# fdarmon/wild_deep_mvs

Hardware: AMD Instinct MI355X
Metric: cost-volume voxels/sec (BxDxHxW), MVSNet hot path (higher is better)
Workload: dtype bf16

## Files before the change

wild_deep_mvs_amd/csrc/conv3d.hip:

```cpp
#include "conv_common.h"
#include <type_traits>

namespace pscv {

PSCV_PROF_BUFFER(conv)

struct ConvArgs : ConvIO {
    int Di, Hi, Wi, Do, Ho, Wo;
    int cout, epi;
    int ntd, nth, ntw;
    unsigned mg_td, mg_th, mg_tw;
    int nt_total;
};

template <int KIND, int TD, int TH> struct Brick;
template <int TD, int TH> struct Brick<PSCV_CONV_S1, TD, TH> { static constexpr int BD = TD + 2, BH = TH + 2, BW = 18; };
template <int TD, int TH> struct Brick<PSCV_CONV_S2, TD, TH> { static constexpr int BD = 2 * TD + 1, BH = 2 * TH + 1, BW = 33; };
template <int TD, int TH> struct Brick<PSCV_CONV_T2, TD, TH> { static constexpr int BD = TD + 1, BH = TH + 1, BW = 17; };

__host__ __device__ constexpr int ceil_div(int a, int b) { return (a + b - 1) / b; }
__host__ __device__ constexpr int t2_ntaps(int pc) { return (1 + ((pc >> 2) & 1)) * (1 + ((pc >> 1) & 1)) * (1 + (pc & 1)); }
__host__ __device__ constexpr int t2_nsteps(int pc, int cin) { return ceil_div(t2_ntaps(pc) * cin, 32); }
__host__ __device__ constexpr int t2_stepbase(int pc, int cin) {
    int s = 0;
    for (int i = 0; i < pc; ++i) s += t2_nsteps(i, cin);
    return s;
}
__host__ __device__ constexpr int conv_total_steps(int kind, int cin) {
    return kind == PSCV_CONV_T2 ? t2_stepbase(8, cin) : ceil_div(27 * cin, 32);
}

__host__ __device__ constexpr int conv_vs(int kind, int cin, int th = 4) {
    if (kind == PSCV_CONV_S1 && cin == 64 && th == 8) return 144;
    if (kind == PSCV_CONV_S2) return cin == 32 ? 80 : cin * 2 + 16;
    return cin == 16 ? 32 : cin == 8 ? 48 : cin * 2 + 32;
}
__host__ __device__ constexpr int conv_epi_bytes(int nt) { return 3 * nt * 16 * 4; }

__host__ __device__ constexpr int conv_region0(int kind, int cin, int nt, int td, int th) {
    const int bd = kind == PSCV_CONV_S1 ? td + 2 : kind == PSCV_CONV_S2 ? 2 * td + 1 : td + 1;
    const int bh = kind == PSCV_CONV_S1 ? th + 2 : kind == PSCV_CONV_S2 ? 2 * th + 1 : th + 1;
    const int bw = kind == PSCV_CONV_S1 ? 18 : kind == PSCV_CONV_S2 ? 33 : 17;
    const int brick = (bd * bh * bw * conv_vs(kind, cin, th) + 15) & ~15;
    const int red = (td * th == 4 && kind != PSCV_CONV_T2) ? 16 * 1024 * nt : 0;
    return brick > red ? brick : red;
}

template <int KIND, int BH, int BW, int VS> __device__ __forceinline__ int tap_off_dense(int tap) {
    tap = tap > 26 ? 26 : tap;
    const int kd = tap / 9, kh = (tap / 3) % 3, kw = tap % 3;
    return ((kd * BH + kh) * BW + kw) * VS;
}
template <int BH, int BW, int VS> __device__ __forceinline__ int tap_off_t2(int pc, int t) {
    const int pd = (pc >> 2) & 1, ph = (pc >> 1) & 1, pw = pc & 1;
    const int nt = (1 + pd) * (1 + ph) * (1 + pw);
    t = t >= nt ? nt - 1 : t;
    const int tw = t % (1 + pw), th = (t / (1 + pw)) % (1 + ph), td = t / ((1 + pw) * (1 + ph));
    const int od = (pd && td == 0) ? 1 : 0, oh = (ph && th == 0) ? 1 : 0, ow = (pw && tw == 0) ? 1 : 0;
    return ((od * BH + oh) * BW + ow) * VS;
}

template <typename H>
__device__ __noinline__ void epi_ragged(float y0, float y1, float y2, float y3, const uint16_t* sp, void* op, int cnt, int out_f32,
                                        float lo_post) {
    float y[4] = {y0, y1, y2, y3};
    for (int k = 0; k < cnt; ++k) {
        float v = y[k];
        if (sp) v += Half16<H>::one(sp[k]);
        v = relu_floor(v, lo_post);
        if (out_f32) reinterpret_cast<float*>(op)[k] = v;
        else reinterpret_cast<uint16_t*>(op)[k] = Half16<H>::bits(v);
    }
}

template <typename H, int CIN, int NT, int KIND, int TD, int TH>
__global__ __launch_bounds__(256) void conv3d_kernel(const ConvArgs a) {
    using BR = Brick<KIND, TD, TH>;
    constexpr int BD = BR::BD, BH = BR::BH, BW = BR::BW;
    constexpr int VS = conv_vs(KIND, CIN, TH);
    constexpr int CCH = CIN / 8;
    constexpr int NVOX = BD * BH * BW;
    constexpr int NMT = TD * TH;
    constexpr int MB = NMT / 4;
    static_assert(NMT % 4 == 0, "tile rows must split evenly over the 4 waves");
    constexpr int SXY = (KIND == PSCV_CONV_S2) ? 2 : 1;

    extern __shared__ __attribute__((aligned(16))) unsigned char smem[];
    PSCV_PROF_BEGIN

    int wg = xcd_remap(blockIdx.x, gridDim.x);
    const int tw_i = fast_divmod(wg, a.ntw, a.mg_tw);
    const int th_i = fast_divmod(wg, a.nth, a.mg_th);
    const int td_i = fast_divmod(wg, a.ntd, a.mg_td);
    const int b = wg;

    const int t0d = td_i * TD, t0h = th_i * TH, t0w = tw_i * 16;
    const int o_d = (KIND == PSCV_CONV_S1) ? t0d - 1 : (KIND == PSCV_CONV_S2) ? 2 * t0d - 1 : t0d;
    const int o_h = (KIND == PSCV_CONV_S1) ? t0h - 1 : (KIND == PSCV_CONV_S2) ? 2 * t0h - 1 : t0h;
    const int o_w = (KIND == PSCV_CONV_S1) ? t0w - 1 : (KIND == PSCV_CONV_S2) ? 2 * t0w - 1 : t0w;

    const int tid = threadIdx.x;
    const int lane = tid & 63, wave = __builtin_amdgcn_readfirstlane(tid >> 6);
    const int n = lane & 15, g = lane >> 4;
    const int nt0 = blockIdx.y * NT;
    const uint4* wpk = reinterpret_cast<const uint4*>(a.wpk);
    constexpr int NSTEPS_ALL = conv_total_steps(KIND, CIN);
    constexpr bool KSPLIT = MB == 1 && KIND != PSCV_CONV_T2;
    constexpr bool CSPLIT = MB == 1 && KIND == PSCV_CONV_T2;
    constexpr int SPW = (NSTEPS_ALL + 3) / 4;
    constexpr int PF_WANT = 24 / NT;
    constexpr int PF_SRC = KSPLIT ? SPW : NSTEPS_ALL;
    constexpr int PF = (KIND == PSCV_CONV_T2) ? 1 : (PF_SRC < PF_WANT ? PF_SRC : PF_WANT);
    uint4 wring[PF][NT];
    if (KIND != PSCV_CONV_T2) {
#pragma unroll
        for (int s = 0; s < PF; ++s) {
            int st = KSPLIT ? wave + 4 * s : s;
            st = st < NSTEPS_ALL ? st : NSTEPS_ALL - 1;
#pragma unroll
            for (int m = 0; m < NT; ++m) wring[s][m] = wpk[(st * a.nt_total + nt0 + m) * 64 + lane];
        }
    }
    constexpr int CS_MAXW = CSPLIT ? t2_nsteps(0, CIN) + t2_nsteps(7, CIN) : 1;
    uint4 wcls[CS_MAXW][NT];
    uint2 skc[CSPLIT ? 8 : 1][NT];
    constexpr int XS = KIND == PSCV_CONV_T2 ? 2 : 1;
    const int ox0 = XS * (t0w + n);
    const int cg = nt0 * 16 + g * 4;
    const unsigned lane_out = (unsigned)(ox0 * a.out_cs + cg), lane_skip = (unsigned)(ox0 * a.skip_cs + cg);
    const bool lane_ok = t0w + n < (KIND == PSCV_CONV_T2 ? a.Wi : a.Wo);
    const long plane_out = (long)a.Ho * a.Wo * a.out_cs, plane_skip = (long)a.Ho * a.Wo * a.skip_cs;
    const int row_out = a.Wo * a.out_cs, row_skip = a.Wo * a.skip_cs;
    const int bDo = b * a.Do;
    const bool cout4 = (a.cout & 3) == 0;
    auto out_row = [&](int od, int oh) -> long { return (long)(bDo + od) * plane_out + (long)oh * row_out + a.out_co; };
    auto skip_row = [&](int od, int oh) -> long { return (long)(bDo + od) * plane_skip + (long)oh * row_skip + a.skip_co; };
    auto skip_fetch = [&](long srow, int pw, int m) -> uint2 {
        uint2 sv = make_uint2(0u, 0u);
        if (a.skip && cout4) {
            if (lane_ok && cg + m * 16 < a.cout)
                sv = *reinterpret_cast<const uint2*>(a.skip + srow + (lane_skip + (unsigned)(pw * a.skip_cs + m * 16)));
        }
        return sv;
    };
    const long cs_orow0 = CSPLIT ? out_row(2 * t0d, 2 * t0h) : 0, cs_srow0 = CSPLIT ? skip_row(2 * t0d, 2 * t0h) : 0;
    auto cls_fetch = [&](auto pcc, auto woffc, auto soffc) {
        constexpr int pc = decltype(pcc)::value, WOFF = decltype(woffc)::value, SOFF = decltype(soffc)::value;
        constexpr int nsteps = t2_nsteps(pc, CIN), sbase = t2_stepbase(pc, CIN);
#pragma unroll
        for (int s = 0; s < nsteps; ++s)
#pragma unroll
            for (int m = 0; m < NT; ++m) wcls[WOFF + s][m] = wpk[((sbase + s) * a.nt_total + nt0 + m) * 64 + lane];
        constexpr int pd = (pc >> 2) & 1, ph = (pc >> 1) & 1, pw = pc & 1;
#pragma unroll
        for (int i = 0; i < 4; ++i) {
            const int id = t0d + i / TH, ih = t0h + i % TH;
            const bool in_ok = id < a.Di && ih < a.Hi;
#pragma unroll
            for (int m = 0; m < NT; ++m)
                skc[SOFF + i][m] = in_ok ? skip_fetch(cs_srow0 + (pd ? plane_skip : 0) + (2 * i + ph) * row_skip, pw, m) : make_uint2(0u, 0u);
        }
    };
    if constexpr (CSPLIT) {
        using std::integral_constant;
#define PSCV_CLS_PAIR(W) case W: cls_fetch(integral_constant<int, W>{}, integral_constant<int, 0>{}, integral_constant<int, 0>{}); \
                             cls_fetch(integral_constant<int, 7 - W>{}, integral_constant<int, t2_nsteps(W, CIN)>{}, integral_constant<int, 4>{}); break;
        switch (wave) { PSCV_CLS_PAIR(0) PSCV_CLS_PAIR(1) PSCV_CLS_PAIR(2) default: PSCV_CLS_PAIR(3) }
#undef PSCV_CLS_PAIR
    }
    uint2 skk[NT];
    if constexpr (KSPLIT) {
#pragma unroll
        for (int m = 0; m < NT; ++m) {
            const int od = t0d + wave / TH, oh = t0h + wave % TH;
            skk[m] = (od < a.Do && oh < a.Ho) ? skip_fetch(skip_row(od, oh), 0, m) : make_uint2(0u, 0u);
        }
    }
    PSCV_STAMP(5)

    {
        constexpr int PC = BH * BW * CCH;
        constexpr int NS = (PC + 255) / 256;
        constexpr int PG = (16 / NS) < 1 ? 1 : ((16 / NS) > BD ? BD : (16 / NS));
        const unsigned long plane_bytes = (unsigned long)a.Hi * a.Wi * a.in_cs * 2;
        const char* inb = reinterpret_cast<const char*>(a.in + (long)b * a.Di * a.Hi * a.Wi * a.in_cs + a.in_co);
        unsigned goff[NS];
        int lds_off[NS];
        bool ok[NS];
#pragma unroll
        for (int sl = 0; sl < NS; ++sl) {
            const int c = sl * 256 + tid;
            const int v = c / CCH, cc = c - v * CCH;
            const int bh = v / BW, bw = v - bh * BW;
            const int gh = o_h + bh, gw = o_w + bw;
            ok[sl] = c < PC && (unsigned)gh < (unsigned)a.Hi && (unsigned)gw < (unsigned)a.Wi;
            goff[sl] = ok[sl] ? (unsigned)(gh * a.Wi + gw) * (unsigned)(a.in_cs * 2) + (unsigned)(cc * 16) : 0u;
            lds_off[sl] = c < PC ? v * VS + cc * 16 : -1;
        }
#pragma unroll
        for (int p0 = 0; p0 < BD; p0 += PG) {
            uint4 val[PG][NS];
#pragma unroll
            for (int pp = 0; pp < PG; ++pp) {
                const int gd = o_d + p0 + pp;
                const bool pv = p0 + pp < BD && (unsigned)gd < (unsigned)a.Di;
                const char* pb = inb + (unsigned long)(pv ? gd : 0) * plane_bytes;
#pragma unroll
                for (int sl = 0; sl < NS; ++sl) {
                    val[pp][sl] = make_uint4(0u, 0u, 0u, 0u);
                    if (pv && ok[sl]) val[pp][sl] = *reinterpret_cast<const uint4*>(pb + goff[sl]);
                }
            }
            PSCV_STAMP(0)
            PSCV_STAMP_WAIT(1)
// ... 217 lines not shown
                    const int koff = tap_off_t2<BH, BW, VS>(pc, kk0 / CIN) + (kk0 % CIN) * 2;
                    const int fs = sbase + s;
                    uint4 wf[NT];
#pragma unroll
                    for (int m = 0; m < NT; ++m) wf[m] = wpk[(fs * a.nt_total + nt0 + m) * 64 + lane];
#pragma unroll
                    for (int i = 0; i < MB; ++i) {
                        const uint4 xf = *reinterpret_cast<const uint4*>(smem + anchor[i] + koff);
#pragma unroll
                        for (int m = 0; m < NT; ++m) acc[i][m] = Mfma<H>::run(wf[m], xf, acc[i][m]);
                    }
                }
            }
            PSCV_STAMP(3)
#pragma unroll
            for (int i = 0; i < MB; ++i) {
                const int mt = wave * MB + i;
                const int id = t0d + mt / TH, ih = t0h + mt % TH;
                if (id < a.Di && ih < a.Hi) epilogue(acc[i], 2 * id + pd, 2 * ih + ph, pw, skp[i]);
            }
            PSCV_STAMP(4)
        }
    }
    PSCV_STAMP_WAIT(5)
    PSCV_PROF_END(conv, blockIdx.x + gridDim.x * blockIdx.y)
}

template <typename H, int CIN, int NT, int KIND, int TD, int TH>
static int launch_conv(ConvArgs& a, int n_split, hipStream_t st) {
    constexpr int LDS = conv_region0(KIND, CIN, NT, TD, TH) + conv_epi_bytes(NT);
    static_assert(LDS <= 160 * 1024, "brick does not fit the 160 KiB LDS");
    const int rd = KIND == PSCV_CONV_T2 ? a.Di : a.Do, rh = KIND == PSCV_CONV_T2 ? a.Hi : a.Ho,
              rw = KIND == PSCV_CONV_T2 ? a.Wi : a.Wo;
    a.ntd = ceil_div(rd, TD); a.nth = ceil_div(rh, TH); a.ntw = ceil_div(rw, 16);
    const long nblk = finish_grid("pscv_conv3d", a.B, a.ntd, a.nth, a.ntw, a.mg_td, a.mg_th, a.mg_tw);
    if (nblk < 0) return -1;
    return launch("pscv_conv3d", conv3d_kernel<H, CIN, NT, KIND, TD, TH>, dim3((unsigned)nblk, (unsigned)n_split), dim3(256), LDS, st, a);
}

template <typename H, int CIN, int NT>
static int launch_kind(ConvArgs& a, int kind, hipStream_t st) {
    a.nt_total = NT;
    const int rd = kind == PSCV_CONV_T2 ? a.Di : a.Do, rh = kind == PSCV_CONV_T2 ? a.Hi : a.Ho,
              rw = kind == PSCV_CONV_T2 ? a.Wi : a.Wo;
    const int TDb = kind == PSCV_CONV_S1 ? 4 : 2, THb = kind == PSCV_CONV_S2 ? 2 : 4;
    const long big = (long)a.B * ceil_div(rd, TDb) * ceil_div(rh, THb) * ceil_div(rw, 16);
    const bool small = big < 1024 && g_conv_small_tiles && kind != PSCV_CONV_S2;
    const int want = (int)g_conv_small_nt;
    auto nts_of = [&](int dflt) { return (want == 1 || want == 2 || want == 4) && want <= NT && NT % want == 0 ? want : dflt; };
#define PSCV_NTS_SWITCH(NTSV, KINDV, TDV, THV)                                                                     \
    switch (NTSV) {                                                                                                  \
        case 1: return launch_conv<H, CIN, 1, KINDV, TDV, THV>(a, NT, st);                                           \
        case 2: if constexpr (NT >= 2) return launch_conv<H, CIN, 2, KINDV, TDV, THV>(a, NT / 2, st); break;         \
        default: if constexpr (NT >= 4) return launch_conv<H, CIN, 4, KINDV, TDV, THV>(a, NT / 4, st); break;        \
    }
    switch (kind) {
        case PSCV_CONV_S1:
            if (small) { PSCV_NTS_SWITCH(nts_of(NT == 2 ? 2 : 1), PSCV_CONV_S1, 1, 4) }
            if constexpr (CIN == 64) {
                if (g_conv_tall64 == 2 || (g_conv_tall64 && (long)a.B * ceil_div(rd, 4) * ceil_div(rh, 8) * ceil_div(rw, 16) >= 256))
                    return launch_conv<H, CIN, NT, PSCV_CONV_S1, 4, 8>(a, 1, st);
            }
            return launch_conv<H, CIN, NT, PSCV_CONV_S1, 4, 4>(a, 1, st);
        case PSCV_CONV_S2: { PSCV_NTS_SWITCH(nts_of(NT), PSCV_CONV_S2, 2, 2) } break;
        case PSCV_CONV_T2:
            if (small) { PSCV_NTS_SWITCH(nts_of(1), PSCV_CONV_T2, 1, 4) }
            return launch_conv<H, CIN, NT, PSCV_CONV_T2, 2, 4>(a, 1, st);
    }
#undef PSCV_NTS_SWITCH
    set_error("pscv_conv3d: unknown kind %d", kind);
    return -1;
}

template <typename H>
static int launch_channels(ConvArgs& a, int c_in, int c_out, int kind, hipStream_t st) {
    const int nt = (c_out + 15) / 16;
#define PSCV_CONV_CASE(CI, NTV) if (c_in == CI && nt == NTV) return launch_kind<H, CI, NTV>(a, kind, st);
    PSCV_CONV_CASE(8, 1) PSCV_CONV_CASE(8, 2)
    PSCV_CONV_CASE(16, 1) PSCV_CONV_CASE(16, 2)
    PSCV_CONV_CASE(32, 1) PSCV_CONV_CASE(32, 2) PSCV_CONV_CASE(32, 4)
    PSCV_CONV_CASE(64, 2) PSCV_CONV_CASE(64, 4)
#undef PSCV_CONV_CASE
    set_error("pscv_conv3d: unsupported channel combination c_in=%d c_out=%d", c_in, c_out);
    return -1;
}

}

PSCV_PROF_EXPORT(conv)

extern "C" int pscv_conv3d_cat2(const void* in_a, int a_cstride, int a_coff, const void* in_b, int b_cstride, int b_coff, int dtype,
                                const uint16_t* packed, const float* scale, const float* bias, const float* floor, const void* skip,
                                int skip_cstride, int skip_coff, void* out, int out_cstride, int out_coff, int out_dtype, int B, int D,
                                int H, int W, int c_out, int epi_flags, void* stream) {
    using namespace pscv;
    PSCV_CHECK_ARG(in_a && in_b && packed && out, "pscv_conv3d_cat2: null pointer argument");
    PSCV_CHECK_ARG(B > 0 && D > 0 && H > 0 && W > 0, "pscv_conv3d_cat2: bad sizes");
    PSCV_CHECK_ARG(c_out == 8 || c_out == 16, "pscv_conv3d_cat2: c_out=%d must be 8 or 16", c_out);
    PSCV_CHECK_ARG(a_cstride % 8 == 0 && a_coff % 8 == 0 && a_coff + 8 <= a_cstride && b_cstride % 8 == 0 && b_coff % 8 == 0 && b_coff + 8 <= b_cstride,
                   "pscv_conv3d_cat2: both inputs contribute an 8-aligned slice of 8 channels");
    PSCV_CHECK_ARG(out_coff + c_out <= out_cstride && out_cstride % 4 == 0 && out_coff % 4 == 0, "pscv_conv3d_cat2: bad output channel slice");
    PSCV_CHECK_ARG(!skip || (skip_cstride % 4 == 0 && skip_coff % 4 == 0), "pscv_conv3d_cat2: skip slice must be 4-aligned");
    PSCV_CHECK_ARG(dtype == PSCV_BF16 || dtype == PSCV_F16, "pscv_conv3d_cat2: storage dtype %d must be bf16 or fp16", dtype);
    PSCV_CHECK_ARG(out_dtype == dtype || out_dtype == PSCV_F32, "pscv_conv3d_cat2: out dtype %d must be the storage dtype or fp32", out_dtype);
    ConvCall c{};
    c.io = {reinterpret_cast<const uint16_t*>(in_a), packed, scale, bias, floor, reinterpret_cast<const uint16_t*>(skip), out,
            a_cstride, a_coff, skip_cstride, skip_coff, out_cstride, out_coff, out_dtype == PSCV_F32, B};
    c.dtype = dtype; c.D = D; c.H = H; c.W = W; c.c_in = 16; c.c_out = c_out; c.epi = epi_flags;
    c.st = reinterpret_cast<hipStream_t>(stream);
    c.in2 = reinterpret_cast<const uint16_t*>(in_b); c.in2_cs = b_cstride; c.in2_co = b_coff;
    return conv3d_sweepc_launch(c);
}

extern "C" int pscv_conv3d(const void* in, int dtype, int in_cstride, int in_coff, const uint16_t* packed, const float* scale,
                           const float* bias, const float* floor, const void* skip, int skip_cstride, int skip_coff,
                           void* out, int out_cstride, int out_coff, int out_dtype, int B, int Di, int Hi, int Wi,
                           int c_in, int c_out, int kind, int epi_flags, void* stream) {
    using namespace pscv;
    PSCV_CHECK_ARG(in && packed && out, "pscv_conv3d: null pointer argument");
    PSCV_CHECK_ARG(B > 0 && Di > 0 && Hi > 0 && Wi > 0, "pscv_conv3d: bad sizes");
    PSCV_CHECK_ARG(in_cstride % 8 == 0 && in_coff % 8 == 0 && in_coff + c_in <= in_cstride,
                   "pscv_conv3d: input channel slice [%d,%d) of stride %d must be 8-aligned", in_coff, in_coff + c_in, in_cstride);
    PSCV_CHECK_ARG(out_coff + c_out <= out_cstride, "pscv_conv3d: output channel slice exceeds stride");
    PSCV_CHECK_ARG(c_out < 4 || (out_cstride % 4 == 0 && out_coff % 4 == 0), "pscv_conv3d: output slice must be 4-aligned");
    PSCV_CHECK_ARG(!skip || c_out < 4 || (skip_cstride % 4 == 0 && skip_coff % 4 == 0), "pscv_conv3d: skip slice must be 4-aligned");
    PSCV_CHECK_ARG(dtype == PSCV_BF16 || dtype == PSCV_F16, "pscv_conv3d: storage dtype %d must be bf16 or fp16", dtype);
    PSCV_CHECK_ARG(out_dtype == dtype || out_dtype == PSCV_F32, "pscv_conv3d: out dtype %d must be the storage dtype or fp32", out_dtype);
    ConvCall c{};
    c.io = {reinterpret_cast<const uint16_t*>(in), packed, scale, bias, floor, reinterpret_cast<const uint16_t*>(skip), out,
            in_cstride, in_coff, skip_cstride, skip_coff, out_cstride, out_coff, out_dtype == PSCV_F32, B};
    c.dtype = dtype; c.D = Di; c.H = Hi; c.W = Wi; c.c_in = c_in; c.c_out = c_out; c.epi = epi_flags;
    c.st = reinterpret_cast<hipStream_t>(stream);
    if (kind == PSCV_CONV_S1P8) {
        PSCV_CHECK_ARG(((c_in == 8 || c_in == 16 || c_in == 32) && c_out == 8) || (c_in == 16 && c_out == 16),
                       "pscv_conv3d: the sweep kernels (S1P8) are for 8|16|32 -> 8 and 16 -> 16 (got %d -> %d)", c_in, c_out);
        return c_in == 32 ? conv3d_sweep8_launch(c) : conv3d_sweepc_launch(c);
    }
    if (kind == PSCV_CONV_T2P8) {
        PSCV_CHECK_ARG(c_in == 16 && c_out == 8, "pscv_conv3d: the parity-pair kernel (T2P8) is for c_in=16, c_out=8 (got %d -> %d)", c_in, c_out);
        return conv3d_t2p8_launch(c);
    }
    if (kind == PSCV_CONV_S1C1) {
        PSCV_CHECK_ARG(c_out == 1 && (c_in == 8 || c_in == 16), "pscv_conv3d: the 1-channel kernel (S1C1) is for c_in 8/16 -> 1 (got %d -> %d)", c_in, c_out);
        return conv3d_c1_launch(c);
    }
    if (kind == PSCV_CONV_S2) {
        const int rc = conv3d_sweep_s2_launch(c);
        if (rc != 1) return rc;
    }
    if (kind == PSCV_CONV_S1) {
        const int rc = conv3d_wide_launch(c);
        if (rc != 1) return rc;
    }
    ConvArgs a;
    static_cast<ConvIO&>(a) = c.io;
    a.Di = Di; a.Hi = Hi; a.Wi = Wi;
    if (kind == PSCV_CONV_S1) { a.Do = Di; a.Ho = Hi; a.Wo = Wi; }
    else if (kind == PSCV_CONV_S2) { a.Do = (Di + 1) / 2; a.Ho = (Hi + 1) / 2; a.Wo = (Wi + 1) / 2; }
    else { a.Do = 2 * Di; a.Ho = 2 * Hi; a.Wo = 2 * Wi; }
    a.cout = c_out; a.epi = epi_flags;
    return with_half("pscv_conv3d", dtype, [&](auto t) { return launch_channels<typename decltype(t)::type>(a, c_in, c_out, kind, c.st); });
}
```

wild_deep_mvs_amd/csrc/conv_common.h:

```cpp
#pragma once
#include "pscv_common.h"

namespace pscv {

struct ConvIO {
    const uint16_t* in;
    const uint16_t* wpk;
    const float* scale;
    const float* bias;
    const float* floor;
    const uint16_t* skip;
    void* out;
    int in_cs, in_co, skip_cs, skip_co, out_cs, out_co;
    int out_f32;
    int B;
};
static_assert(sizeof(ConvIO) == 88, "7 pointers + 8 ints: the kernels' own fields follow at byte 88");

struct ConvCall {
    ConvIO io;
    int dtype;
    int D, H, W;
    int c_in, c_out, epi;
    hipStream_t st;
    const uint16_t* in2;
    int in2_cs, in2_co;
};

struct HeadOut {
    const float* depth;
    long depth_bstride;
    float* part;
    long part_floats;
    float *o_depth, *o_conf;
    float *o_index, *o_entropy;
};

int conv3d_sweep8_launch(const ConvCall& c);
int conv3d_sweepc_launch(const ConvCall& c);
int conv3d_sweep_s2_launch(const ConvCall& c);
int conv3d_wide_launch(const ConvCall& c);
int conv3d_c1_launch(const ConvCall& c);
int conv3d_t2p8_launch(const ConvCall& c);
void softargmin_merge_launch(const ConvCall& c, const HeadOut& h, int ndc);

inline int plan_depth_chunk(int D, long tiles, long slots, int min_dc, bool even, int forced) {
    const long ndc_want = tiles >= slots ? 1 : slots / tiles;
    int dc = (int)((D + ndc_want - 1) / ndc_want);
    if (even) dc = (dc + 1) & ~1;
    dc = dc < min_dc ? min_dc : dc;
    if (forced > 0) dc = even ? forced & ~1 : forced;
    return dc > D ? (even ? (D + 1) & ~1 : D) : dc;
}

inline long finish_grid(const char* what, int B, int n0, int n1, int n2, unsigned& mg0, unsigned& mg1, unsigned& mg2) {
    mg0 = fast_div_magic(n0); mg1 = fast_div_magic(n1); mg2 = fast_div_magic(n2);
    const long nblk = (long)B * n0 * n1 * n2;
    if (nblk <= 0 || nblk > 0x7fffffffL) { set_error("%s: bad grid %ld", what, nblk); return -1; }
    return nblk;
}

}
```

wild_deep_mvs_amd/csrc/pscv_common.h:

```cpp
#pragma once
#include <hip/hip_runtime.h>
#include <stdint.h>
#include <stdio.h>
#include <stdarg.h>

#include "../../include/pscv.h"

namespace pscv {

void set_error(const char* fmt, ...);

hipError_t ensure_dyn_lds(const void* kernel, int bytes);
int device_cu_count();

struct Knob {
    int process;
    int id;
    operator int() const;
    void set(int v) { __atomic_store_n(&process, v, __ATOMIC_RELAXED); }
};
#define PSCV_KNOB_TABLE(X)                      \
    X("warp_q2", g_warp_q2, 1)                  \
    X("warp_lpv", g_warp_lpv_override, 0)       \
    X("warp_ppd", g_warp_ppd_override, 0)       \
    X("warp_tiled", g_warp_tiled, 1)            \
    X("warp_tile", g_warp_tile, 0)              \
    X("warp_gc_lds", g_warp_gc_lds, 1)          \
    X("warp_lds_pad", g_warp_lds_pad, 0)        \
    X("warp_bwd_direct", g_warp_bwd_direct, 0)  \
    X("sweep_dc", g_sweep_dc, 0)                \
    X("sweepc_slots", g_sweepc_slots, 0)        \
    X("sweepc_pd", g_sweepc_pd, 0)              \
    X("sweep_th16", g_sweep_th16, 0)            \
    X("sweep_kdm", g_sweep_kdm, 0)              \
    X("sweep_kdm_pd", g_sweep_kdm_pd, 0)        \
    X("c1_sweep", g_c1_sweep, 1)                \
    X("c1_nb", g_c1_nb, 0)                      \
    X("conv_s2_sweep", g_conv_s2_sweep, 1)      \
    X("s2s_slots", g_s2s_slots, 0)              \
    X("block8_slots", g_block8_slots, 0)        \
    X("conv2d_wlds", g_conv2d_wlds, 1)          \
    X("conv_wide", g_conv_wide, 1)              \
    X("conv_tall64", g_conv_tall64, 1)          \
    X("conv_small_tiles", g_conv_small_tiles, 1) \
    X("conv_small_nt", g_conv_small_nt, 0)      \
    X("tail_nbk", g_tail_nbk, 0)                \
    X("softargmin_small", g_softargmin_small, 1) \
    X("fuse_c0", g_fuse_c0, 0)
#define PSCV_KNOB_DECLARE(key, sym, def) extern Knob sym;
PSCV_KNOB_TABLE(PSCV_KNOB_DECLARE)
#undef PSCV_KNOB_DECLARE

#define PSCV_CHECK_ARG(cond, ...)          \
    do {                                   \
        if (!(cond)) {                     \
            pscv::set_error(__VA_ARGS__);  \
            return -1;                     \
        }                                  \
    } while (0)

#define PSCV_CHECK_LAUNCH(name)                                                        \
    do {                                                                               \
        hipError_t e_ = hipGetLastError();                                             \
        if (e_ != hipSuccess) {                                                        \
            pscv::set_error("%s: launch failed: %s", name, hipGetErrorString(e_));     \
            return -2;                                                                 \
        }                                                                              \
    } while (0)

constexpr size_t DYN_LDS_OPT_IN = 60000;
int dyn_lds_opt_in(const char* what, const void* kernel, size_t lds);
int launch_status(const char* what);

template <typename... KArgs, typename... Args>
int launch(const char* what, void (*kern)(KArgs...), dim3 grid, dim3 block, size_t lds, hipStream_t st, Args&&... args) {
    if (lds > DYN_LDS_OPT_IN) {
        const int rc = dyn_lds_opt_in(what, reinterpret_cast<const void*>(kern), lds);
        if (rc) return rc;
    }
    hipLaunchKernelGGL(kern, grid, block, lds, st, static_cast<KArgs>(args)...);
    return launch_status(what);
}

#ifdef PSCV_PROFILE
constexpr int PSCV_PROF_BLOCKS = 16384;
#define PSCV_PROF_BUFFER(tag) __device__ unsigned int pscv_prof_##tag[pscv::PSCV_PROF_BLOCKS * 16];
#define PSCV_PROF_BEGIN unsigned long long pt_prev = __builtin_readcyclecounter(); const unsigned long long pt_begin = pt_prev; \
    unsigned pt_acc[6] = {0, 0, 0, 0, 0, 0};
#define PSCV_STAMP(i) { const unsigned long long t_ = __builtin_readcyclecounter(); pt_acc[i] += (unsigned)(t_ - pt_prev); pt_prev = t_; }
#define PSCV_STAMP_WAIT(i) { asm volatile("s_waitcnt vmcnt(0) lgkmcnt(0)" ::: "memory"); PSCV_STAMP(i) }
#define PSCV_PROF_END(tag, blk) if (threadIdx.x == 0 && (blk) < pscv::PSCV_PROF_BLOCKS) { \
        unsigned hwid_, xcc_; asm volatile("s_getreg_b32 %0, hwreg(HW_REG_HW_ID)" : "=s"(hwid_)); \
        asm volatile("s_getreg_b32 %0, hwreg(HW_REG_XCC_ID)" : "=s"(xcc_)); \
        unsigned int* o_ = pscv_prof_##tag + (blk) * 16; \
        for (int i_ = 0; i_ < 6; ++i_) o_[i_] = pt_acc[i_]; \
        o_[6] = (unsigned)pt_begin; o_[7] = (unsigned)pt_prev; o_[8] = hwid_; o_[9] = xcc_; }
#define PSCV_PROF_EXPORT(tag) extern "C" int pscv_debug_prof_##tag(unsigned int* out, int n_blocks) { \
        if (n_blocks > pscv::PSCV_PROF_BLOCKS) n_blocks = pscv::PSCV_PROF_BLOCKS; \
        return (int)hipMemcpyFromSymbol(out, HIP_SYMBOL(pscv::pscv_prof_##tag), (size_t)n_blocks * 16 * sizeof(unsigned int)); }
#else
#define PSCV_PROF_BUFFER(tag)
#define PSCV_PROF_BEGIN
#define PSCV_STAMP(i)
#define PSCV_STAMP_WAIT(i)
#define PSCV_PROF_END(tag, blk)
#define PSCV_PROF_EXPORT(tag)
#endif

__host__ __device__ __forceinline__ unsigned fast_div_magic(int d) { return d <= 1 ? 0u : (unsigned)((1ull << 32) / (unsigned)d) + 1u; }
__device__ __forceinline__ int fast_divmod(int& x, int d, unsigned mg) {
    unsigned q = d <= 1 ? (unsigned)x : __umulhi((unsigned)x, mg);
    int r = x - (int)(q * (unsigned)d);
    if (r < 0) { --q; r += d; }
    x = (int)q;
    return r;
}

__device__ __forceinline__ int xcd_run(int xcd, int n, int& end) {
    const int q = n >> 3, r = n & 7;
    const int first = xcd < r ? xcd * (q + 1) : r * (q + 1) + (xcd - r) * q;
    end = first + q + (xcd < r ? 1 : 0);
    return first;
}
__device__ __forceinline__ int xcd_remap(int bid, int nwg) {
    int end;
    return xcd_run(bid & 7, nwg, end) + (bid >> 3);
}

__host__ __device__ __forceinline__ float bf16_to_f32(uint16_t v) {
    union { uint32_t u; float f; } c;
    c.u = ((uint32_t)v) << 16;
    return c.f;
}
__host__ __device__ __forceinline__ uint16_t f32_to_bf16(float f) {
    union { uint32_t u; float f; } c;
    c.f = f;
    uint32_t u = c.u;
    if ((u & 0x7fffffffu) > 0x7f800000u) return (uint16_t)((u >> 16) | 0x40);
    u += 0x7fffu + ((u >> 16) & 1u);
    return (uint16_t)(u >> 16);
}
typedef __bf16 bf16x2_hw_t __attribute__((ext_vector_type(2)));
__device__ __forceinline__ uint32_t pack_bf16x2(float lo, float hi) {
    bf16x2_hw_t v;
    v[0] = (__bf16)lo;
    v[1] = (__bf16)hi;
    return __builtin_bit_cast(uint32_t, v);
}
__device__ __forceinline__ float bf16lo(uint32_t x) { return __uint_as_float(x << 16); }
__device__ __forceinline__ float bf16hi(uint32_t x) { return __uint_as_float(x & 0xffff0000u); }

__host__ __device__ __forceinline__ uint16_t f32_to_f16_bits(float f) {
    union { uint32_t u; float f; } c;
    c.f = f;
    const uint32_t sign = (c.u >> 16) & 0x8000u;
    uint32_t x = c.u & 0x7fffffffu;
    if (x > 0x7f800000u) return (uint16_t)(sign | 0x7e00u);
    if (x > 0x477fe000u) return (uint16_t)(sign | 0x7bffu);
    if (x < 0x38800000u) {
        if (x < 0x33000000u) return (uint16_t)sign;
        const uint32_t mant = (x & 0x7fffffu) | 0x800000u;
        const int shift = 126 - (int)(x >> 23);
        uint32_t h = mant >> shift;
        const uint32_t rem = mant & ((1u << shift) - 1u), halfway = 1u << (shift - 1);
        if (rem > halfway || (rem == halfway && (h & 1u))) ++h;
        return (uint16_t)(sign | h);
    }
    uint32_t h = (x - 0x38000000u) >> 13;
    const uint32_t rem = x & 0x1fffu;
    if (rem > 0x1000u || (rem == 0x1000u && (h & 1u))) ++h;
    return (uint16_t)(sign | h);
}
typedef _Float16 h2_t __attribute__((ext_vector_type(2)));
__device__ __forceinline__ float f16lo(uint32_t x) { return (float)__builtin_bit_cast(h2_t, x)[0]; }
__device__ __forceinline__ float f16hi(uint32_t x) { return (float)__builtin_bit_cast(h2_t, x)[1]; }
__device__ __forceinline__ uint32_t pack_f16x2(float lo, float hi) {
    h2_t v;
    v[0] = (_Float16)__builtin_amdgcn_fmed3f(lo, -65504.0f, 65504.0f);
    v[1] = (_Float16)__builtin_amdgcn_fmed3f(hi, -65504.0f, 65504.0f);
    return __builtin_bit_cast(uint32_t, v);
}

__device__ __forceinline__ void fp16_ovfl_mode(bool on = true) {
    __builtin_amdgcn_sched_barrier(0);
    if (on) __builtin_amdgcn_s_setreg((1 - 1) << 11 | 23 << 6 | 1, 1);
    else __builtin_amdgcn_s_setreg((1 - 1) << 11 | 23 << 6 | 1, 0);
    __builtin_amdgcn_sched_barrier(0);
}
__device__ __forceinline__ uint32_t pack_f16x2_ovfl(float lo, float hi) {
    h2_t v;
    v[0] = (_Float16)lo;
    v[1] = (_Float16)hi;
    return __builtin_bit_cast(uint32_t, v);
}
__device__ __forceinline__ float relu_floor(float x, float lo) { return x < lo ? lo : x; }
__device__ __forceinline__ float clamp_lo(float x, float lo) { return relu_floor(x, lo); }

struct bf16_t { uint16_t bits; };
// ... 107 lines not shown
```

Baseline: 13.53 billion.

## Add depth-sweeping transposed-conv kernel with LDS plane ring and parity-paired waves

```diff
diff --git a/wild_deep_mvs_amd/csrc/conv3d.hip b/wild_deep_mvs_amd/csrc/conv3d.hip
--- a/wild_deep_mvs_amd/csrc/conv3d.hip
+++ b/wild_deep_mvs_amd/csrc/conv3d.hip
@@ -18,23 +18,10 @@
 template <int TD, int TH> struct Brick<PSCV_CONV_S2, TD, TH> { static constexpr int BD = 2 * TD + 1, BH = 2 * TH + 1, BW = 33; };
 template <int TD, int TH> struct Brick<PSCV_CONV_T2, TD, TH> { static constexpr int BD = TD + 1, BH = TH + 1, BW = 17; };
 
-__host__ __device__ constexpr int ceil_div(int a, int b) { return (a + b - 1) / b; }
-__host__ __device__ constexpr int t2_ntaps(int pc) { return (1 + ((pc >> 2) & 1)) * (1 + ((pc >> 1) & 1)) * (1 + (pc & 1)); }
-__host__ __device__ constexpr int t2_nsteps(int pc, int cin) { return ceil_div(t2_ntaps(pc) * cin, 32); }
-__host__ __device__ constexpr int t2_stepbase(int pc, int cin) {
-    int s = 0;
-    for (int i = 0; i < pc; ++i) s += t2_nsteps(i, cin);
-    return s;
-}
 __host__ __device__ constexpr int conv_total_steps(int kind, int cin) {
     return kind == PSCV_CONV_T2 ? t2_stepbase(8, cin) : ceil_div(27 * cin, 32);
 }
 
-__host__ __device__ constexpr int conv_vs(int kind, int cin, int th = 4) {
-    if (kind == PSCV_CONV_S1 && cin == 64 && th == 8) return 144;
-    if (kind == PSCV_CONV_S2) return cin == 32 ? 80 : cin * 2 + 16;
-    return cin == 16 ? 32 : cin == 8 ? 48 : cin * 2 + 32;
-}
 __host__ __device__ constexpr int conv_epi_bytes(int nt) { return 3 * nt * 16 * 4; }
 
 __host__ __device__ constexpr int conv_region0(int kind, int cin, int nt, int td, int th) {
@@ -51,15 +38,6 @@
     const int kd = tap / 9, kh = (tap / 3) % 3, kw = tap % 3;
     return ((kd * BH + kh) * BW + kw) * VS;
 }
-template <int BH, int BW, int VS> __device__ __forceinline__ int tap_off_t2(int pc, int t) {
-    const int pd = (pc >> 2) & 1, ph = (pc >> 1) & 1, pw = pc & 1;
-    const int nt = (1 + pd) * (1 + ph) * (1 + pw);
-    t = t >= nt ? nt - 1 : t;
-    const int tw = t % (1 + pw), th = (t / (1 + pw)) % (1 + ph), td = t / ((1 + pw) * (1 + ph));
-    const int od = (pd && td == 0) ? 1 : 0, oh = (ph && th == 0) ? 1 : 0, ow = (pw && tw == 0) ? 1 : 0;
-    return ((od * BH + oh) * BW + ow) * VS;
-}
-
 template <typename H>
 __device__ __noinline__ void epi_ragged(float y0, float y1, float y2, float y3, const uint16_t* sp, void* op, int cnt, int out_f32,
                                         float lo_post) {
@@ -583,6 +561,10 @@
         const int rc = conv3d_wide_launch(c);
         if (rc != 1) return rc;
     }
+    if (kind == PSCV_CONV_T2) {
+        const int rc = conv3d_t2sweep_launch(c);
+        if (rc != 1) return rc;
+    }
     ConvArgs a;
     static_cast<ConvIO&>(a) = c.io;
     a.Di = Di; a.Hi = Hi; a.Wi = Wi;
diff --git a/wild_deep_mvs_amd/csrc/conv3d_t2sweep.hip b/wild_deep_mvs_amd/csrc/conv3d_t2sweep.hip
--- /dev/null
+++ b/wild_deep_mvs_amd/csrc/conv3d_t2sweep.hip
@@ -0,0 +1,226 @@
+#include "conv_common.h"
+#include <type_traits>
+
+namespace pscv {
+
+struct T2SweepArgs : ConvIO {
+    int Di, Hi, Wi;
+    int epi;
+    int dc, ndc, nth, ntw;
+    unsigned mg_dc, mg_th, mg_tw;
+    int nt_total;
+};
+
+constexpr int TS_TH = 4, TS_BH = TS_TH + 1, TS_BW = 17;
+constexpr int TS_NT = 512, TS_RW = 2;
+template <int V> using ic = std::integral_constant<int, V>;
+typedef unsigned int ts_u32x2 __attribute__((ext_vector_type(2)));
+PSCV_PROF_BUFFER(t2sweep)
+
+template <typename H, int CIN>
+__global__ __launch_bounds__(TS_NT) void conv3d_t2sweep_kernel(const T2SweepArgs a) {
+    constexpr int VS = conv_vs(PSCV_CONV_T2, CIN);
+    constexpr int CCH = CIN / 8;
+    constexpr int PLANE = TS_BH * TS_BW * VS;
+    constexpr int PC = TS_BH * TS_BW * CCH;
+    constexpr int NS = (PC + TS_NT - 1) / TS_NT;
+    constexpr int MAXW = t2_nsteps(0, CIN) + t2_nsteps(7, CIN);
+    static_assert(CIN % 32 == 0, "a k-step holds 32 channels of one tap");
+    static_assert(PLANE % 16 == 0 && 3 * PLANE <= 64 * 1024, "ring slots are 16-byte aligned and fit the static LDS");
+    __shared__ __attribute__((aligned(16))) unsigned char ring[3 * PLANE];
+    PSCV_PROF_BEGIN
+
+    int wg = xcd_remap(blockIdx.x, gridDim.x);
+    const int tw_i = fast_divmod(wg, a.ntw, a.mg_tw);
+    const int th_i = fast_divmod(wg, a.nth, a.mg_th);
+    const int dc_i = fast_divmod(wg, a.ndc, a.mg_dc);
+    const int b = wg;
+    const int t0h = th_i * TS_TH, t0w = tw_i * 16;
+    const int d0 = dc_i * a.dc, d1 = min(d0 + a.dc, a.Di);
+
+    const int tid = threadIdx.x;
+    const int lane = tid & 63, wave8 = __builtin_amdgcn_readfirstlane(tid >> 6);
+    const int wave = wave8 & 3, r0 = (wave8 >> 2) * TS_RW;
+    const int n = lane & 15, g = lane >> 4;
+    const int nt0 = blockIdx.y;
+    const int Do = 2 * a.Di, Ho = 2 * a.Hi, Wo = 2 * a.Wi;
+
+    const int cg = nt0 * 16 + g * 4;
+    const bool lane_ok = t0w + n < a.Wi;
+    const unsigned out_row_b = (unsigned)Wo * a.out_cs * 2, out_plane_b = (unsigned)Ho * out_row_b, out_vol_b = (unsigned)Do * out_plane_b;
+    const unsigned sk_row_b = (unsigned)Wo * a.skip_cs * 2, sk_plane_b = (unsigned)Ho * sk_row_b, sk_vol_b = (unsigned)Do * sk_plane_b;
+    char* const outb = reinterpret_cast<char*>(a.out) + ((unsigned long)b * out_vol_b + (unsigned long)a.out_co * 2);
+    const char* const skb = reinterpret_cast<const char*>(a.skip) + ((unsigned long)b * sk_vol_b + (unsigned long)a.skip_co * 2);
+    const int out_sz = (int)(out_vol_b - (unsigned)a.out_co * 2), sk_sz = a.skip ? (int)(sk_vol_b - (unsigned)a.skip_co * 2) : 0;
+    unsigned out_voff[2], sk_voff[2];
+#pragma unroll
+    for (int pw = 0; pw < 2; ++pw) {
+        const int ox = 2 * (t0w + n) + pw;
+        out_voff[pw] = lane_ok ? (unsigned)(ox * a.out_cs + cg) * 2u : 0x7ffffff0u;
+        sk_voff[pw] = lane_ok ? (unsigned)(ox * a.skip_cs + cg) * 2u : 0x7ffffff0u;
+    }
+    const unsigned out_row0 = (unsigned)(2 * t0h) * out_row_b, sk_row0 = (unsigned)(2 * t0h) * sk_row_b;
+
+    const uint4* wpk = reinterpret_cast<const uint4*>(a.wpk);
+    uint4 wcls[MAXW];
+    auto cls_weights = [&](auto pcc, auto woffc, auto, auto, int, int, int) {
+        constexpr int pc = decltype(pcc)::value, WOFF = decltype(woffc)::value;
+        constexpr int nsteps = t2_nsteps(pc, CIN), sbase = t2_stepbase(pc, CIN);
+#pragma unroll
+        for (int s = 0; s < nsteps; ++s) wcls[WOFF + s] = wpk[((sbase + s) * a.nt_total + nt0) * 64 + lane];
+    };
+    uint2 skc[2][2 * TS_RW];
+    auto cls_skips = [&](auto pcc, auto, auto soffc, auto par, int i, int, int) {
+        constexpr int pc = decltype(pcc)::value, SOFF = decltype(soffc)::value, PAR = decltype(par)::value;
+        constexpr int pd = (pc >> 2) & 1, ph = (pc >> 1) & 1, pw = pc & 1;
+        const bool pl_ok = i < d1;
+        const unsigned sp = (unsigned)(2 * i + pd) * sk_plane_b + sk_row0;
+#pragma unroll
+        for (int r = 0; r < TS_RW; ++r) {
+            const __amdgpu_buffer_rsrc_t rs = __builtin_amdgcn_make_buffer_rsrc(const_cast<char*>(skb), (short)0, (pl_ok && t0h + r0 + r < a.Hi) ? sk_sz : 0, 0x00020000);
+            skc[PAR][SOFF + r] = __builtin_bit_cast(uint2, __builtin_amdgcn_raw_buffer_load_b64(rs, (int)sk_voff[pw], (int)(sp + (unsigned)(2 * (r0 + r) + ph) * sk_row_b), 0));
+        }
+    };
+#define PSCV_TS_PAIR(W, F, P, I, CUR, NXT) F(ic<W>{}, ic<0>{}, ic<0>{}, P, I, CUR, NXT); F(ic<7 - W>{}, ic<t2_nsteps(W, CIN)>{}, ic<TS_RW>{}, P, I, CUR, NXT); break;
+#define PSCV_TS_ROLE(F, P, I, CUR, NXT)                                                                                         \
+    switch (wave) { case 0: PSCV_TS_PAIR(0, F, P, I, CUR, NXT) case 1: PSCV_TS_PAIR(1, F, P, I, CUR, NXT)                       \
+                    case 2: PSCV_TS_PAIR(2, F, P, I, CUR, NXT) default: PSCV_TS_PAIR(3, F, P, I, CUR, NXT) }
+
+    float sc[4], bi[4], fl[4];
+#pragma unroll
+    for (int k = 0; k < 4; ++k) {
+        sc[k] = a.scale ? a.scale[cg + k] : 1.0f;
+        bi[k] = a.bias ? a.bias[cg + k] : 0.0f;
+        fl[k] = (a.epi & PSCV_EPI_RELU_PRE) ? (a.floor ? a.floor[cg + k] : 0.0f) : -__builtin_inff();
+    }
+    const float lo_post = (a.epi & PSCV_EPI_RELU_POST) ? 0.0f : -__builtin_inff();
+
+    const unsigned in_plane_b = (unsigned)a.Hi * a.Wi * a.in_cs * 2;
+    const unsigned in_plane_sz = in_plane_b - (unsigned)a.in_co * 2;
+    const char* inb = reinterpret_cast<const char*>(a.in) + ((unsigned long)b * a.Di * in_plane_b + (unsigned long)a.in_co * 2);
+    unsigned goff[NS];
+    int loff[NS];
+#pragma unroll
+    for (int sl = 0; sl < NS; ++sl) {
+        const int c = sl * TS_NT + tid;
+        const int v = c / CCH, cc = c - v * CCH;
+        const int bh = v / TS_BW, bw = v - bh * TS_BW;
+        const int gh = t0h + bh, gw = t0w + bw;
+        const bool ok = c < PC && gh < a.Hi && gw < a.Wi;
+        goff[sl] = ok ? (unsigned)(gh * a.Wi + gw) * (unsigned)(a.in_cs * 2) + (unsigned)(cc * 16) : 0x7ffffff0u;
+        loff[sl] = c < PC ? v * VS + cc * 16 : -1;
+    }
+    auto ifetch = [&](int plane, uint4 (&reg)[NS]) {
+        const bool pv = plane < a.Di && plane <= d1;
+        const __amdgpu_buffer_rsrc_t rs = __builtin_amdgcn_make_buffer_rsrc(
+            const_cast<char*>(inb + (unsigned long)(pv ? plane : 0) * in_plane_b), (short)0, pv ? (int)in_plane_sz : 0, 0x00020000);
+#pragma unroll
+        for (int sl = 0; sl < NS; ++sl) reg[sl] = __builtin_bit_cast(uint4, __builtin_amdgcn_raw_buffer_load_b128(rs, (int)goff[sl], 0, 0));
+    };
+    auto istash = [&](int slot, const uint4 (&reg)[NS]) {
+        unsigned char* sp = ring + slot * PLANE;
+#pragma unroll
+        for (int sl = 0; sl < NS; ++sl)
+            if (loff[sl] >= 0) *reinterpret_cast<uint4*>(sp + loff[sl]) = reg[sl];
+    };
+
+    const int lane_lds = (r0 * TS_BW + n) * VS + g * 16;
+    auto cls_run = [&](auto pcc, auto woffc, auto soffc, auto par, int i, int cur, int nxt) {
+        constexpr int pc = decltype(pcc)::value, WOFF = decltype(woffc)::value, SOFF = decltype(soffc)::value, PAR = decltype(par)::value;
+        constexpr int nsteps = t2_nsteps(pc, CIN);
+        constexpr int pd = (pc >> 2) & 1, ph = (pc >> 1) & 1, pw = pc & 1;
+        f32x4 acc[TS_RW];
+#pragma unroll
+        for (int r = 0; r < TS_RW; ++r) acc[r] = f32x4{0.f, 0.f, 0.f, 0.f};
+#pragma unroll
+        for (int s = 0; s < nsteps; ++s) {
+            const int off = tap_off_t2<TS_BH, TS_BW, VS>(pc, (s * 32) / CIN) + ((s * 32) % CIN) * 2;
+            const bool up = off >= PLANE;
+            const unsigned char* bp = ring + (up ? nxt : cur) + (up ? off - PLANE : off) + lane_lds;
+#pragma unroll
+            for (int r = 0; r < TS_RW; ++r) {
+                const uint4 xf = *reinterpret_cast<const uint4*>(bp + r * (TS_BW * VS));
+                acc[r] = Mfma<H>::run(wcls[WOFF + s], xf, acc[r]);
+            }
+        }
+        PSCV_STAMP(3)
+        const unsigned op = (unsigned)(2 * i + pd) * out_plane_b + out_row0;
+#pragma unroll
+        for (int r = 0; r < TS_RW; ++r) {
+            float y[4];
+#pragma unroll
+            for (int k = 0; k < 4; ++k) y[k] = relu_floor(fmaf(acc[r][k], sc[k], bi[k]), fl[k]);
+            const uint2 sv = skc[PAR][SOFF + r];
+            y[0] = relu_floor(y[0] + Half16<H>::lo(sv.x), lo_post); y[1] = relu_floor(y[1] + Half16<H>::hi(sv.x), lo_post);
+            y[2] = relu_floor(y[2] + Half16<H>::lo(sv.y), lo_post); y[3] = relu_floor(y[3] + Half16<H>::hi(sv.y), lo_post);
+            const __amdgpu_buffer_rsrc_t rs = __builtin_amdgcn_make_buffer_rsrc(outb, (short)0, t0h + r0 + r < a.Hi ? out_sz : 0, 0x00020000);
+            __builtin_amdgcn_raw_buffer_store_b64(__builtin_bit_cast(ts_u32x2, make_uint2(Half16<H>::pack(y[0], y[1]), Half16<H>::pack(y[2], y[3]))), rs,
+                                                  (int)out_voff[pw], (int)(op + (unsigned)(2 * (r0 + r) + ph) * out_row_b), 0);
+        }
+        PSCV_STAMP(4)
+    };
+    uint4 val[NS];
+    {
+        uint4 v0[NS], v1[NS];
+        PSCV_TS_ROLE(cls_skips, ic<0>{}, d0, 0, 0)
+        PSCV_TS_ROLE(cls_weights, ic<0>{}, 0, 0, 0)
+        ifetch(d0, v0);
+        ifetch(d0 + 1, v1);
+        ifetch(d0 + 2, val);
+        PSCV_STAMP(5)
+        istash(0, v0);
+        istash(1, v1);
+    }
+    auto plane_step = [&](auto par, const int i, const int s_cur) {
+        constexpr int PAR = decltype(par)::value;
+        const int s_nxt = s_cur == 2 ? 0 : s_cur + 1, s_nn = s_cur == 0 ? 2 : s_cur - 1;
+        PSCV_TS_ROLE(cls_skips, ic<1 - PAR>{}, i + 1, 0, 0)
+        PSCV_STAMP(0)
+        __syncthreads();
+        PSCV_STAMP(2)
+        PSCV_TS_ROLE(cls_run, par, i, s_cur * PLANE, s_nxt * PLANE)
+        istash(s_nn, val);
+        ifetch(i + 3, val);
+        PSCV_STAMP(1)
+    };
+    int i = d0, slot = 0;
+    for (; i + 1 < d1; i += 2) {
+        plane_step(ic<0>{}, i, slot);
+        slot = slot == 2 ? 0 : slot + 1;
+        plane_step(ic<1>{}, i + 1, slot);
+        slot = slot == 2 ? 0 : slot + 1;
+    }
+    if (i < d1) plane_step(ic<0>{}, i, slot);
+#undef PSCV_TS_ROLE
+#undef PSCV_TS_PAIR
+    PSCV_PROF_END(t2sweep, blockIdx.x + gridDim.x * blockIdx.y)
+}
+
+int conv3d_t2sweep_launch(const ConvCall& c) {
+    const ConvIO& io = c.io;
+    if (!g_t2_sweep) return 1;
+    if (!((c.c_in == 32 && c.c_out == 16) || (c.c_in == 64 && c.c_out == 32))) return 1;
+    if (io.out_f32 || (c.dtype != PSCV_BF16 && c.dtype != PSCV_F16)) return 1;
+    if ((io.out_cs | io.out_co) & 3 || (io.skip && ((io.skip_cs | io.skip_co) & 3))) return 1;
+    const long vox = (long)c.D * c.H * c.W;
+    if (vox * io.in_cs * 2 >= 0x7ffffff0L || 8 * vox * io.out_cs * 2 >= 0x7ffffff0L || (io.skip && 8 * vox * io.skip_cs * 2 >= 0x7ffffff0L)) return 1;
+    T2SweepArgs a;
+    static_cast<ConvIO&>(a) = io;
+    a.Di = c.D; a.Hi = c.H; a.Wi = c.W; a.epi = c.epi;
+    a.nth = ceil_div(c.H, TS_TH); a.ntw = ceil_div(c.W, 16); a.nt_total = c.c_out / 16;
+    const int n_cu = device_cu_count();
+    if (n_cu <= 0) { set_error("pscv_conv3d(t2sweep): device query failed"); return -2; }
+    a.dc = plan_depth_chunk(c.D, (long)a.B * a.nth * a.ntw * a.nt_total, n_cu, 2, false, g_sweep_dc);
+    a.ndc = ceil_div(c.D, a.dc);
+    const long nblk = finish_grid("pscv_conv3d(t2sweep)", a.B, a.ndc, a.nth, a.ntw, a.mg_dc, a.mg_th, a.mg_tw);
+    if (nblk < 0) return -1;
+    return with_half("pscv_conv3d(t2sweep)", c.dtype, [&](auto t) {
+        using H = typename decltype(t)::type;
+        if (c.c_in == 32) return launch("pscv_conv3d(t2sweep)", conv3d_t2sweep_kernel<H, 32>, dim3((unsigned)nblk, (unsigned)a.nt_total), dim3(TS_NT), 0, c.st, a);
+        return launch("pscv_conv3d(t2sweep)", conv3d_t2sweep_kernel<H, 64>, dim3((unsigned)nblk, (unsigned)a.nt_total), dim3(TS_NT), 0, c.st, a);
+    });
+}
+
+}
+
+PSCV_PROF_EXPORT(t2sweep)
diff --git a/wild_deep_mvs_amd/csrc/conv_common.h b/wild_deep_mvs_amd/csrc/conv_common.h
--- a/wild_deep_mvs_amd/csrc/conv_common.h
+++ b/wild_deep_mvs_amd/csrc/conv_common.h
@@ -42,7 +42,32 @@
 int conv3d_wide_launch(const ConvCall& c);
 int conv3d_c1_launch(const ConvCall& c);
 int conv3d_t2p8_launch(const ConvCall& c);
+int conv3d_t2sweep_launch(const ConvCall& c);
 void softargmin_merge_launch(const ConvCall& c, const HeadOut& h, int ndc);
+
+__host__ __device__ constexpr int ceil_div(int a, int b) { return (a + b - 1) / b; }
+__host__ __device__ constexpr int t2_ntaps(int pc) { return (1 + ((pc >> 2) & 1)) * (1 + ((pc >> 1) & 1)) * (1 + (pc & 1)); }
+__host__ __device__ constexpr int t2_nsteps(int pc, int cin) { return ceil_div(t2_ntaps(pc) * cin, 32); }
+__host__ __device__ constexpr int t2_stepbase(int pc, int cin) {
+    int s = 0;
+    for (int i = 0; i < pc; ++i) s += t2_nsteps(i, cin);
+    return s;
+}
+
+__host__ __device__ constexpr int conv_vs(int kind, int cin, int th = 4) {
+    if (kind == PSCV_CONV_S1 && cin == 64 && th == 8) return 144;
+    if (kind == PSCV_CONV_S2) return cin == 32 ? 80 : cin * 2 + 16;
+    return cin == 16 ? 32 : cin == 8 ? 48 : cin * 2 + 32;
+}
+
+template <int BH, int BW, int VS> __device__ __forceinline__ int tap_off_t2(int pc, int t) {
+    const int pd = (pc >> 2) & 1, ph = (pc >> 1) & 1, pw = pc & 1;
+    const int nt = (1 + pd) * (1 + ph) * (1 + pw);
+    t = t >= nt ? nt - 1 : t;
+    const int tw = t % (1 + pw), th = (t / (1 + pw)) % (1 + ph), td = t / ((1 + pw) * (1 + ph));
+    const int od = (pd && td == 0) ? 1 : 0, oh = (ph && th == 0) ? 1 : 0, ow = (pw && tw == 0) ? 1 : 0;
+    return ((od * BH + oh) * BW + ow) * VS;
+}
 
 inline int plan_depth_chunk(int D, long tiles, long slots, int min_dc, bool even, int forced) {
     const long ndc_want = tiles >= slots ? 1 : slots / tiles;
diff --git a/wild_deep_mvs_amd/csrc/pscv_common.h b/wild_deep_mvs_amd/csrc/pscv_common.h
--- a/wild_deep_mvs_amd/csrc/pscv_common.h
+++ b/wild_deep_mvs_amd/csrc/pscv_common.h
@@ -44,6 +44,7 @@
     X("conv_tall64", g_conv_tall64, 1)          \
     X("conv_small_tiles", g_conv_small_tiles, 1) \
     X("conv_small_nt", g_conv_small_nt, 0)      \
+    X("t2_sweep", g_t2_sweep, 1)                \
     X("tail_nbk", g_tail_nbk, 0)                \
     X("softargmin_small", g_softargmin_small, 1) \
     X("fuse_c0", g_fuse_c0, 0)
```

After: 13.52 billion. Within noise of the previous version (-0.1%).
